# montyhall/bot7

Hardware: NVIDIA B200
Metric: EI candidates scored/s at N=4096, S=32 hypers (higher is better)
Workload: dtype f64

## Files before the change

bot7_b200/csrc/posterior_i8.cu:

```cuda
#include <math.h>
#include <stdlib.h>

#include "b7_internal.h"
#include "exp_neg.cuh"
#include "gemm_tile.cuh"
#include "i8_common.cuh"

using b7g::mbar_init; using b7g::mbar_wait; using b7g::mbar_arrive; using b7g::mbar_arrive_expect_tx; using b7g::bulk_g2s;
using b7g::mbar_fence_init; using b7g::smem_u32;
using namespace b7i8;

namespace {

constexpr int TM = 128, TN = 64, KB = 64;
constexpr int KC = KB / 16;
constexpr int A_STAGE = NS * TM * KB;
constexpr int B_STAGE = NS * TN * KB;
constexpr int STAGE = A_STAGE + B_STAGE;
constexpr int NSTAGE = 2;
static_assert(STAGE % 1024 == 0 && KB % 32 == 0 && 64 % KB == 0, "stage geometry");
static_assert(KB == b7i8::gemm::KB && TM == b7i8::gemm::TM && TN == b7i8::gemm::TN && NSTAGE == b7i8::gemm::NSTAGE,
              "posterior_i8_kernel issues its MMAs through the shared stage of i8_common.cuh");
constexpr int I8_THREADS = 192;
constexpr int RED_BYTES = 2 * 4 * TN * 8;
constexpr int I8_SMEM = NSTAGE * STAGE + RED_BYTES + 1024;
constexpr int TNH = TN / 2;
constexpr int B_HALF = NS * TNH * KB;
constexpr int P_STAGE = A_STAGE + B_HALF;
constexpr int P_NSTAGE = 3;
constexpr int P_SMEM = P_NSTAGE * P_STAGE + RED_BYTES + 1024;
constexpr int P_THREADS = 320;
static_assert(P_STAGE % 1024 == 0 && P_SMEM <= 227 * 1024, "pair stage geometry");


__host__ __device__ __forceinline__ long long pk_off(int rb) {
  const long long j = rb >> 1;
  return 4 * j * (j + 1) + (rb & 1) * 4 * (j + 1);
}

__global__ void __launch_bounds__(SLICE_THREADS)
slice_factor_kernel(const double* __restrict__ fac, long long fac_stride, int Np, int8_t* __restrict__ facS,
                    long long facS_stride, double* __restrict__ sigma, int s0) {
  __shared__ double s_red[SLICE_THREADS];
  const int rb = blockIdx.x, s = s0 + blockIdx.y, row = threadIdx.x & 127, q = threadIdx.x >> 7;
  const int KTA = Np / 16, NB = Np / TM;
  const int n_kc = rb < NB ? (rb + 1) * (TM / 16) : 0, all_kc = ((rb >> 1) + 1) * 4 * KC;
  int8_t* dst = facS + (long long)s * facS_stride + pk_off(rb) * A_STAGE;
  double inv = 0.0;
  const double* src = fac + (long long)s * fac_stride + b7g::tile_off(KTA, rb < NB ? rb : 0, 0);
  if (rb < NB) {
    double mx = 0.0;
    bool bad = false;
    for (int kc = q; kc < n_kc; kc += 4) chunk_max(src + b7g::elem_off(row, kc * 16), mx, bad);
    const double sg = row_scale(mx, bad, s_red, row, q);
    inv = sg != sg ? 0.0 : 1.0 / sg;
    if (q == 0) sigma[(long long)s * Np + rb * TM + row] = sg;
  }
  for (int kc = q; kc < all_kc; kc += 4) {
    uint32_t pk[4][NS];
    if (kc < n_kc) {
      chunk_digits(src + b7g::elem_off(row, kc * 16), inv, pk);
    } else {
#pragma unroll
      for (int g = 0; g < 4; ++g)
#pragma unroll
        for (int p = 0; p < NS; ++p) pk[g][p] = 0u;
    }
    const int ks = kc / KC, kcc = kc % KC;
#pragma unroll
    for (int p = 0; p < NS; ++p)
      *reinterpret_cast<uint4*>(dst + (long long)ks * A_STAGE + p * (KC * TM * 16) + kcc * (TM * 16) + row * 16) =
          make_uint4(pk[0][p], pk[1][p], pk[2][p], pk[3][p]);
  }
}

template <int DT, int KERNEL, bool PAIR>
__global__ void __launch_bounds__(128)
cov_slices_kernel(const double* __restrict__ A, long long rows, int d, const double* __restrict__ Xt, int N, int Np,
                  const double* __restrict__ par, double inv_tau, const double* __restrict__ alpha, int8_t* __restrict__ ksS,
                  double* __restrict__ meanP) {
  __shared__ __align__(16) double s_x[DT][64];
  __shared__ double s_w[DT];
  __shared__ double s_tab[64];
  __shared__ __align__(16) double s_al[64];
  __shared__ double s_dot[64];
  if (threadIdx.x < 64) s_tab[threadIdx.x] = c_exp_tab[threadIdx.x];
  const int ct = blockIdx.x, kb64 = blockIdx.y, KS_ALL = Np / KB;
  const int c = threadIdx.x & 63;
  for (int e = threadIdx.x; e < DT * 64; e += 128) {
    const int i = e / 64, k = kb64 * 64 + e % 64;
    s_x[i][e % 64] = (i < d && k < N) ? Xt[(long long)i * Np + k] : 0.0;
  }
  if (threadIdx.x >= 64) s_al[c] = alpha[kb64 * 64 + c];
  if (threadIdx.x < DT) s_w[threadIdx.x] = threadIdx.x < d ? par[threadIdx.x] : 0.0;
  __syncthreads();
  const long long row = (long long)ct * TN + c;
  double a[DT];
#pragma unroll
  for (int i = 0; i < DT; ++i) a[i] = (row < rows && i < d) ? A[row * d + i] : 0.0;
  const double sf2s = par[B7_MAX_DIMS] * inv_tau * 18014398509481984.0;
  double dot = 0.0;
  double w[DT];
#pragma unroll
  for (int j = 0; j < DT; ++j) w[j] = s_w[j];
  ExpNegK K;
  K.init();
  const bool live = row < rows;
#pragma unroll 1
  for (int half = 0; half < 2; ++half) {
  const int kc = (threadIdx.x >> 6) + 2 * half;
  uint32_t pk[4][NS];
  unsigned long long z[4];
#pragma unroll
  for (int i = 0; i < 16; i += 2) {
    const int kk = kc * 16 + i, k = kb64 * 64 + kk;
    double r2a = 0.0, r2b = 0.0;
#pragma unroll
    for (int j = 0; j < DT; ++j) {
      const double2 x2 = *reinterpret_cast<const double2*>(&s_x[j][kk]);
      const double ta = (a[j] - x2.x) * w[j], tb = (a[j] - x2.y) * w[j];
      r2a = fma(ta, ta, r2a);
      r2b = fma(tb, tb, r2b);
    }
    double va, vb;
    if (KERNEL == B7_KERNEL_ARDSE) {
      va = sf2s * exp_neg_k(-0.5 * r2a, s_tab, K);
      vb = sf2s * exp_neg_k(-0.5 * r2b, s_tab, K);
    } else {
      const double ra = sqrt(r2a), s5a = 2.23606797749978969641 * ra, rb = sqrt(r2b), s5b = 2.23606797749978969641 * rb;
      va = sf2s * ((1.0 + s5a + (5.0 / 3.0) * r2a) * exp_neg_k(-s5a, s_tab, K));
      vb = sf2s * ((1.0 + s5b + (5.0 / 3.0) * r2b) * exp_neg_k(-s5b, s_tab, K));
    }
    va = (live && k < N) ? va : 0.0;
    vb = (live && k + 1 < N) ? vb : 0.0;
    const double2 al = *reinterpret_cast<const double2*>(&s_al[kk]);
    dot = fma(va, al.x, dot);
    dot = fma(vb, al.y, dot);
    z[i & 3] = digit_bytes_scaled(va);
    z[(i & 3) + 1] = digit_bytes_scaled(vb);
    if ((i & 3) == 2) pack4(z, pk[i >> 2]);
  }
  const int gkc = kb64 * 4 + kc, ks = gkc / KC, kcc = gkc % KC;
  int8_t* dst = PAIR ? ksS + (((long long)ct * KS_ALL + ks) * 2 + (c >> 5)) * B_HALF + kcc * (TNH * 16) + (c & 31) * 16
                     : ksS + ((long long)ct * KS_ALL + ks) * B_STAGE + kcc * (TN * 16) + c * 16;
  constexpr int P_STRIDE = PAIR ? KC * TNH * 16 : KC * TN * 16;
#pragma unroll
  for (int p = 0; p < NS; ++p) *reinterpret_cast<uint4*>(dst + p * P_STRIDE) = make_uint4(pk[0][p], pk[1][p], pk[2][p], pk[3][p]);
  }
  if (threadIdx.x >= 64) s_dot[c] = dot;
  __syncthreads();
  if (threadIdx.x < 64) meanP[((long long)ct * (Np / 64) + kb64) * 64 + c] = dot + s_dot[c];
}

__device__ __forceinline__ double lane_transpose_sum(double (&x)[32], int lane) {
#pragma unroll
  for (int s = 16; s >= 1; s >>= 1) {
    const bool up = (lane & s) != 0;
#pragma unroll
    for (int j = 0; j < s; ++j) {
      const double send = up ? x[j] : x[j + s];
      const double keep = up ? x[j + s] : x[j];
      x[j] = keep + __shfl_xor_sync(0xffffffffu, send, s);
    }
  }
  return x[0];
}

struct Walk {
  int NB, chunk, group, n_tiles;
  __device__ __forceinline__ int cpt() const { return (NB + chunk - 1) / chunk; }
  __device__ __forceinline__ int npl() const { return (cpt() + 1) / 2; }
  __device__ __forceinline__ int n_items() const { return n_tiles * npl(); }
  __device__ __forceinline__ int grp(int item) const {
    const int g = item / (group * npl()), last = (n_tiles - 1) / group;
    return g < last ? g : last;
  }
  __device__ __forceinline__ int g_tiles(int g) const { return n_tiles - g * group < group ? n_tiles - g * group : group; }
  __device__ __forceinline__ int tile(int item) const {
    const int g = grp(item);
    return g * group + (item - g * group * npl()) % g_tiles(g);
  }
  __device__ __forceinline__ int level(int item) const {
    const int g = grp(item);
    return (item - g * group * npl()) / g_tiles(g);
  }
  __device__ __forceinline__ int parts(int item) const { return 2 * level(item) == cpt() - 1 ? 1 : 2; }
  __device__ __forceinline__ int rb_begin(int item, int part) const { return (part == 0 ? level(item) : cpt() - 1 - level(item)) * chunk; }
  __device__ __forceinline__ int rb_end(int item, int part) const {
    const int e = rb_begin(item, part) + chunk;
    return e < NB ? e : NB;
  }
};


template <typename F>
__device__ __forceinline__ void epilogue_row_block(uint32_t tmem, int tid, int warp, int lane, double sc, double* rr, double* out,
                                                   F arrive_drained) {
  double v[TN];
  b7i8::gemm::drain_classes(tmem, warp, v);
  tc_fence_before();
  __syncwarp();
  if (lane == 0) arrive_drained();
#pragma unroll
  for (int h = 0; h < 2; ++h) {
    double x[32];
#pragma unroll
    for (int c = 0; c < 32; ++c) { const double vv = v[h * 32 + c] * sc; x[c] = vv * vv; }
    rr[warp * TN + h * 32 + lane] = lane_transpose_sum(x, lane);
  }
  asm volatile("bar.sync 1, 128;\n" ::: "memory");
  if (tid < TN && out) out[tid] = ((rr[0 * TN + tid] + rr[1 * TN + tid]) + rr[2 * TN + tid]) + rr[3 * TN + tid];
}

template <typename F>
__device__ __forceinline__ void epilogue_row_block8(uint32_t tmem, int tid, int warp, int lane, double sc, double* rr, double* out,
                                                    F arrive_drained) {
  const int q = warp & 3, hc = warp >> 2;
  const uint32_t base = tmem + ((uint32_t)(q * 32) << 16) + (uint32_t)(hc * 32);
  double v[32];
  uint32_t a[4][32];
#pragma unroll
  for (int i = 0; i < 3; ++i) tmem_ld32_async(base + (uint32_t)(i * TN), a[i]);
  tmem_ld_wait();
#pragma unroll
  for (int c = 0; c < 32; ++c) v[c] = 0.0;
#pragma unroll
  for (int i = 0; i < 3; ++i) {
    tmem_pin(a[i]);
    const double wt = ldexp(1.0, 4 - 8 * (i + 2));
#pragma unroll
    for (int c = 0; c < 32; ++c) v[c] = fma((double)(int)a[i][c], wt, v[c]);
  }
#pragma unroll
  for (int i = 0; i < 4; ++i) tmem_ld32_async(base + (uint32_t)((3 + i) * TN), a[i]);
  tmem_ld_wait();
#pragma unroll
  for (int i = 0; i < 4; ++i) tmem_pin(a[i]);
  tc_fence_before();
  __syncwarp();
  if (lane == 0) arrive_drained();
#pragma unroll
  for (int i = 0; i < 4; ++i) {
    const double wt = ldexp(1.0, 4 - 8 * (i + 5));
#pragma unroll
    for (int c = 0; c < 32; ++c) v[c] = fma((double)(int)a[i][c], wt, v[c]);
  }
#pragma unroll
  for (int c = 0; c < 32; ++c) { const double vv = v[c] * sc; v[c] = vv * vv; }
  rr[q * TN + hc * 32 + lane] = lane_transpose_sum(v, lane);
  asm volatile("bar.sync 1, 256;\n" ::: "memory");
  if (tid < TN && out) out[tid] = ((rr[0 * TN + tid] + rr[1 * TN + tid]) + rr[2 * TN + tid]) + rr[3 * TN + tid];
}

__global__ void __launch_bounds__(I8_THREADS, 1)
posterior_i8_kernel(const int8_t* __restrict__ facS, const double* __restrict__ sigma, int Np, int NB,
                    const int8_t* __restrict__ ksS, double tau, int chunk, int group, int n_tiles, double* __restrict__ partial) {
  extern __shared__ __align__(1024) uint8_t smem[];
  double* red = reinterpret_cast<double*>(smem + NSTAGE * STAGE);
  uint64_t* bars = reinterpret_cast<uint64_t*>(smem + NSTAGE * STAGE + RED_BYTES);
  uint64_t *full = bars, *empty = bars + NSTAGE, *acc_full = bars + 2 * NSTAGE, *acc_empty = bars + 2 * NSTAGE + 1;
  uint32_t* tmem_slot = reinterpret_cast<uint32_t*>(bars + 2 * NSTAGE + 2);
  const int tid = threadIdx.x, warp = tid >> 5, lane = tid & 31;
  const int KS_ALL = Np / KB;
  const Walk wk{NB, chunk, group, n_tiles};
  if (tid == 0) {
    for (int s = 0; s < NSTAGE; ++s) { mbar_init(full + s, 1); mbar_init(empty + s, 1); }
    mbar_init(acc_full, 1);
    mbar_init(acc_empty, 4);
    mbar_fence_init();
  }
  if (warp == 4) {
    asm volatile("tcgen05.alloc.cta_group::1.sync.aligned.shared::cta.b32 [%0], %1;\n" ::"r"(smem_u32(tmem_slot)), "n"(512) : "memory");
    asm volatile("tcgen05.relinquish_alloc_permit.cta_group::1.sync.aligned;\n" ::: "memory");
  }
  tc_fence_before();
  __syncthreads();
  tc_fence_after();
  const uint32_t tmem = *tmem_slot;

  if (warp == 4) {
    int slot = 0;
    unsigned phase = 1;
    bool wrapped = false;
    for (int item = blockIdx.x; item < wk.n_items(); item += gridDim.x) {
      const int tile = wk.tile(item);
      const int8_t* gB = ksS + (long long)tile * KS_ALL * B_STAGE;
      for (int part = 0; part < wk.parts(item); ++part)
        for (int rb = wk.rb_begin(item, part); rb < wk.rb_end(item, part); ++rb) {
          const int8_t* gA = facS + pk_off(rb) * A_STAGE;
          for (int ks = 0; ks < (TM / KB) * (rb + 1); ++ks) {
            if (wrapped) mbar_wait(empty + slot, phase);
            if (elect_one()) {
              uint8_t* st = smem + slot * STAGE;
              mbar_arrive_expect_tx(full + slot, STAGE);
              bulk_g2s(st, gA + (long long)ks * A_STAGE, A_STAGE, full + slot);
              bulk_g2s(st + A_STAGE, gB + (long long)ks * B_STAGE, B_STAGE, full + slot);
            }
            __syncwarp();
            if (++slot == NSTAGE) { slot = 0; phase ^= 1u; wrapped = true; }
          }
        }
    }
  } else if (warp == 5) {
    const uint32_t idesc = (2u << 4) | (1u << 7) | (1u << 10) | ((uint32_t)(TN >> 3) << 17) | ((uint32_t)(TM >> 4) << 24);
    int slot = 0, done = 0;
    unsigned phase = 0;
    for (int item = blockIdx.x; item < wk.n_items(); item += gridDim.x)
      for (int part = 0; part < wk.parts(item); ++part)
        for (int rb = wk.rb_begin(item, part); rb < wk.rb_end(item, part); ++rb, ++done) {
          if (done > 0) { mbar_wait(acc_empty, (unsigned)((done - 1) & 1)); tc_fence_after(); }
          const int n_ks = (TM / KB) * (rb + 1);
          for (int ks = 0; ks < n_ks; ++ks) {
            mbar_wait(full + slot, phase);
            tc_fence_after();
            if (elect_one()) {
              b7i8::gemm::mma_stage(smem + slot * STAGE, tmem, idesc, ks == 0);
              umma_commit(empty + slot);
              if (ks == n_ks - 1) umma_commit(acc_full);
            }
            __syncwarp();
            if (++slot == NSTAGE) { slot = 0; phase ^= 1u; }
          }
        }
  } else {
    int done = 0;
    for (int item = blockIdx.x; item < wk.n_items(); item += gridDim.x) {
      const int tile = wk.tile(item);
      for (int part = 0; part < wk.parts(item); ++part)
        for (int rb = wk.rb_begin(item, part); rb < wk.rb_end(item, part); ++rb, ++done) {
          mbar_wait(acc_full, (unsigned)(done & 1));
          tc_fence_after();
          epilogue_row_block(tmem, tid, warp, lane, sigma[rb * TM + tid] * tau, red + (done & 1) * (4 * TN),
                             partial + ((long long)tile * NB + rb) * TN, [&] { mbar_arrive(acc_empty); });
        }
    }
  }
  tc_fence_before();
  __syncthreads();
  if (warp == 4) asm volatile("tcgen05.dealloc.cta_group::1.sync.aligned.b32 %0, %1;\n" ::"r"(tmem), "n"(512) : "memory");
}

__global__ void __cluster_dims__(2, 1, 1) __launch_bounds__(P_THREADS, 1)
posterior_i8_pair_kernel(const int8_t* __restrict__ facS, const double* __restrict__ sigma, int Np, int NB,
                         const int8_t* __restrict__ ksS, double tau, int group, int n_tiles, double* __restrict__ partial, int dbg) {
  extern __shared__ __align__(1024) uint8_t smem[];
  double* red = reinterpret_cast<double*>(smem + P_NSTAGE * P_STAGE);
  uint64_t* bars = reinterpret_cast<uint64_t*>(smem + P_NSTAGE * P_STAGE + RED_BYTES);
  uint64_t *full = bars, *empty = bars + P_NSTAGE, *peer_full = bars + 2 * P_NSTAGE, *acc_full = bars + 3 * P_NSTAGE,
           *acc_empty = bars + 3 * P_NSTAGE + 1;
  uint32_t* tmem_slot = reinterpret_cast<uint32_t*>(bars + 3 * P_NSTAGE + 2);
  const int tid = threadIdx.x, warp = tid >> 5, lane = tid & 31;
  const int KS_ALL = Np / KB;
  const uint32_t rank = cluster_ctarank();
  const int pair_id = blockIdx.x >> 1, n_pairs = gridDim.x >> 1;
  const Walk wk{(NB + 1) / 2, 1, group, n_tiles};
  if (tid == 0) {
    for (int s = 0; s < P_NSTAGE; ++s) { mbar_init(full + s, 1); mbar_init(empty + s, 1); mbar_init(peer_full + s, 1); }
    mbar_init(acc_full, 1);
    mbar_init(acc_empty, 16);
    mbar_fence_init();
  }
  if (warp == 8) {
    asm volatile("tcgen05.alloc.cta_group::2.sync.aligned.shared::cta.b32 [%0], %1;\n" ::"r"(smem_u32(tmem_slot)), "n"(512) : "memory");
    asm volatile("tcgen05.relinquish_alloc_permit.cta_group::2.sync.aligned;\n" ::: "memory");
  }
  tc_fence_before();
  __syncthreads();
  cluster_sync_all();
  tc_fence_after();
  const uint32_t tmem = *tmem_slot;

  if (warp == 8) {
    const uint64_t pol_last = l2_policy_evict_last(), pol_first = l2_policy_evict_first();
    int slot = 0;
    unsigned phase = 1;
    bool wrapped = false;
    for (int item = pair_id; item < wk.n_items(); item += n_pairs) {
      const int tile = wk.tile(item);
      const int8_t* gB = ksS + ((long long)tile * KS_ALL * 2 + rank) * B_HALF;
      for (int part = 0; part < wk.parts(item); ++part)
        for (int j = wk.rb_begin(item, part); j < wk.rb_end(item, part); ++j) {
          const int8_t* gA = facS + pk_off(2 * j + (int)rank) * A_STAGE;
          for (int ks = 0; ks < 4 * (j + 1); ++ks) {
            if (wrapped) mbar_wait_cluster(empty + slot, phase);
            if (elect_one()) {
              uint8_t* st = smem + slot * P_STAGE;
              if (dbg & 4) {
                mbar_arrive_expect_tx(full + slot, 2048);
                bulk_g2s(st, facS, 1024, full + slot);
                bulk_g2s(st + A_STAGE, ksS, 1024, full + slot);
                __syncwarp();
                if (++slot == P_NSTAGE) { slot = 0; phase ^= 1u; wrapped = true; }
                continue;
              }
              mbar_arrive_expect_tx(full + slot, P_STAGE);
              if (dbg & 2) {
                bulk_g2s(st, facS, A_STAGE, full + slot);
                bulk_g2s(st + A_STAGE, ksS, B_HALF, full + slot);
              } else {
                const int hint = dbg >> 4;
                if (hint == 1 || hint == 2) bulk_g2s_hint(st, gA + (long long)ks * A_STAGE, A_STAGE, full + slot, pol_last);
                else if (hint == 4 || hint == 5) bulk_g2s_hint(st, gA + (long long)ks * A_STAGE, A_STAGE, full + slot, pol_first);
                else bulk_g2s(st, gA + (long long)ks * A_STAGE, A_STAGE, full + slot);
                if (hint == 2 || hint == 3) bulk_g2s_hint(st + A_STAGE, gB + (long long)ks * (2 * B_HALF), B_HALF, full + slot, pol_first);
                else if (hint == 4 || hint == 6) bulk_g2s_hint(st + A_STAGE, gB + (long long)ks * (2 * B_HALF), B_HALF, full + slot, pol_last);
                else bulk_g2s(st + A_STAGE, gB + (long long)ks * (2 * B_HALF), B_HALF, full + slot);
              }
            }
            __syncwarp();
            if (++slot == P_NSTAGE) { slot = 0; phase ^= 1u; wrapped = true; }
          }
        }
    }
  } else if (warp == 9) {
    int slot = 0, done = 0;
    unsigned phase = 0;
    if (rank == 0) {
      const uint32_t idesc = (2u << 4) | (1u << 7) | (1u << 10) | ((uint32_t)(TN >> 3) << 17) | ((uint32_t)(256 >> 4) << 24);
      for (int item = pair_id; item < wk.n_items(); item += n_pairs)
        for (int part = 0; part < wk.parts(item); ++part)
          for (int j = wk.rb_begin(item, part); j < wk.rb_end(item, part); ++j, ++done) {
            if (done > 0) { mbar_wait_cluster(acc_empty, (unsigned)((done - 1) & 1)); tc_fence_after(); }
            const int n_ks = 4 * (j + 1);
            for (int ks = 0; ks < n_ks; ++ks) {
              mbar_wait_cluster(full + slot, phase);
              mbar_wait_cluster(peer_full + slot, phase);
              tc_fence_after();
              if (elect_one()) {
                const uint8_t* st = smem + slot * P_STAGE;
                const uint64_t da0 = umma_desc(st, TM * 16, 128), db0 = umma_desc(st + A_STAGE, TNH * 16, 128);
#pragma unroll
                for (int k2 = 0; k2 < KB / 32; ++k2) {
#pragma unroll
                  for (int p = 1; p <= NS; ++p) {
                    const uint64_t da = da0 + (uint64_t)(((p - 1) * (KC * TM * 16) + k2 * (2 * TM * 16)) >> 4);
                    const uint32_t acc = (ks == 0 && k2 == 0 && p == 1) ? 0u : 1u;
                    const int nq = NS + 1 - p;
#pragma unroll
                    for (int q = 1; q <= nq; ++q) {
                      const uint64_t db = db0 + (uint64_t)(((q - 1) * (KC * TNH * 16) + k2 * (2 * TNH * 16)) >> 4);
                      const uint32_t dcol = tmem + (uint32_t)((p + q - 2) * TN);
                      if (nq == 1) umma_i8_pair<0>(dcol, da, db, idesc, acc);
                      else if (q == 1) umma_i8_pair<1>(dcol, da, db, idesc, acc);
                      else if (q == nq) umma_i8_pair<3>(dcol, da, db, idesc, acc);
                      else umma_i8_pair<2>(dcol, da, db, idesc, acc);
                    }
                  }
                }
                umma_commit_pair(empty + slot);
                if (ks == n_ks - 1) umma_commit_pair(acc_full);
              }
              __syncwarp();
              if (++slot == P_NSTAGE) { slot = 0; phase ^= 1u; }
            }
          }
    } else {
      for (int item = pair_id; item < wk.n_items(); item += n_pairs)
        for (int part = 0; part < wk.parts(item); ++part)
          for (int j = wk.rb_begin(item, part); j < wk.rb_end(item, part); ++j)
            for (int ks = 0; ks < 4 * (j + 1); ++ks) {
              mbar_wait_cluster(full + slot, phase);
              if (elect_one()) mbar_arrive_cluster(peer_full + slot, 0);
              __syncwarp();
              if (++slot == P_NSTAGE) { slot = 0; phase ^= 1u; }
            }
    }
  } else {
    int done = 0;
    for (int item = pair_id; item < wk.n_items(); item += n_pairs) {
      const int tile = wk.tile(item);
      for (int part = 0; part < wk.parts(item); ++part)
        for (int j = wk.rb_begin(item, part); j < wk.rb_end(item, part); ++j, ++done) {
          const int rb = 2 * j + (int)rank;
          mbar_wait_cluster(acc_full, (unsigned)(done & 1));
          tc_fence_after();
          if (dbg & 1) {
            tc_fence_before();
            __syncwarp();
            if (lane == 0) mbar_arrive_cluster(acc_empty, 0);
            continue;
          }
          const double sc = rb < NB ? sigma[rb * TM + (tid & 127)] * tau : 0.0;
          epilogue_row_block8(tmem, tid, warp, lane, sc, red + (done & 1) * (4 * TN),
                             rb < NB ? partial + ((long long)tile * NB + rb) * TN : nullptr, [&] { mbar_arrive_cluster(acc_empty, 0); });
        }
    }
  }
  tc_fence_before();
  __syncthreads();
  cluster_sync_all();
  if (warp == 8) asm volatile("tcgen05.dealloc.cta_group::2.sync.aligned.b32 %0, %1;\n" ::"r"(tmem), "n"(512) : "memory");
}

__global__ void __launch_bounds__(128)
posterior_i8_finish_kernel(const double* __restrict__ partial, const double* __restrict__ meanP, int NB, int Np,
                           const double* __restrict__ cand, long long rows, int d, const double* __restrict__ Xt,
                           const double* __restrict__ par, int kernel, double sf2, double mconst, double mean_scale,
                           long long cols_pad, double* __restrict__ mean, double* __restrict__ var) {
  const long long c = (long long)blockIdx.x * blockDim.x + threadIdx.x;
  if (c >= cols_pad) return;
  const double* p = partial + (c / TN) * NB * TN + c % TN;
  double run2 = 0.0, run1 = 0.0;
  for (int rb = 0; rb < NB; ++rb) run2 += p[(long long)rb * TN];
  const double* q = meanP + (c / TN) * (Np / 64) * 64 + c % TN;
  for (int kb = 0; kb < Np / 64; ++kb) run1 += q[(long long)kb * 64];
  double r2 = 0.0;
  if (c < rows)
    for (int j = 0; j < d; ++j) {
      const double t = (cand[c * d + j] - Xt[(long long)j * Np]) * par[j];
      r2 = fma(t, t, r2);
    }
  const bool nan_row = (r2 != r2) || (kernel == B7_KERNEL_MATERN52 && isinf(r2));
  const double poison = nan_row ? __longlong_as_double(0x7ff8000000000000LL) : 0.0;
  const double vv = sf2 - run2;
  var[c] = (vv > 0.0 ? vv : (vv != vv ? vv : 0.0)) + poison;
  mean[c] = (nan_row ? 0.0 : fma(run1, mean_scale, mconst)) + poison;
}

bool g_attr_i8[16] = {false};

}

size_t b7_i8_facs_stride(int Np) {
  const long long P = (Np / TM + 1) / 2;
  return (size_t)(4 * P * (P + 1)) * A_STAGE;
}

int b7_i8_slice_factor(b7_ctx* ctx, const double* fac, int Np, int8_t* facS, double* sigma, int s0, int count) {
  const int NBp = (Np / TM + 1) / 2 * 2;
  slice_factor_kernel<<<dim3(NBp, count), SLICE_THREADS, 0, ctx->stream>>>(fac, (long long)Np * Np, Np, facS, (long long)b7_i8_facs_stride(Np), sigma, s0);
  b7_count(ctx);
  B7_CUDA(cudaGetLastError());
  return 0;
}

template <int DT>
static int launch_cov_slices(b7_ctx* ctx, cudaStream_t st, int kernel, const double* A, int64_t rows, int64_t rows_pad, int d,
                             const double* Xt, int N, int Np, const double* par, double inv_tau, const double* alpha, int8_t* ksS,
                             double* meanP) {
  dim3 grid((unsigned)(rows_pad / TN), Np / 64);
  const bool se = kernel == B7_KERNEL_ARDSE;
  if (ctx->post_pair) {
    if (se) cov_slices_kernel<DT, B7_KERNEL_ARDSE, true><<<grid, 128, 0, st>>>(A, rows, d, Xt, N, Np, par, inv_tau, alpha, ksS, meanP);
    else cov_slices_kernel<DT, B7_KERNEL_MATERN52, true><<<grid, 128, 0, st>>>(A, rows, d, Xt, N, Np, par, inv_tau, alpha, ksS, meanP);
  } else {
    if (se) cov_slices_kernel<DT, B7_KERNEL_ARDSE, false><<<grid, 128, 0, st>>>(A, rows, d, Xt, N, Np, par, inv_tau, alpha, ksS, meanP);
    else cov_slices_kernel<DT, B7_KERNEL_MATERN52, false><<<grid, 128, 0, st>>>(A, rows, d, Xt, N, Np, par, inv_tau, alpha, ksS, meanP);
  }
  b7_count(ctx);
  B7_CUDA(cudaGetLastError());
  return 0;
}

int b7_i8_cov_slices(b7_ctx* ctx, cudaStream_t st, int kernel, const double* A, int64_t rows, int64_t rows_pad, int d, const double* Xt,
                     int N, int Np, const double* par, double tau, const double* alpha, int8_t* ksS, double* meanP) {
  if (rows_pad <= 0) return 0;
  const double inv_tau = 1.0 / tau;
#define B7_COV_SLICES(DT) return launch_cov_slices<DT>(ctx, st, kernel, A, rows, rows_pad, d, Xt, N, Np, par, inv_tau, alpha, ksS, meanP)
  if (d <= 2) B7_COV_SLICES(2);
  if (d <= 4) B7_COV_SLICES(4);
  if (d <= 6) B7_COV_SLICES(6);
  if (d <= 8) B7_COV_SLICES(8);
  if (d <= 12) B7_COV_SLICES(12);
  if (d <= 16) B7_COV_SLICES(16);
  if (d <= 20) B7_COV_SLICES(20);
  if (d <= 24) B7_COV_SLICES(24);
  if (d <= 32) B7_COV_SLICES(32);
  B7_COV_SLICES(40);
#undef B7_COV_SLICES
}

size_t b7_i8_partial_bytes(int Np, int64_t cols_pad) {
  return (size_t)(cols_pad / TN) * ((size_t)(Np / TM) * TN + (size_t)(Np / 64) * 64) * sizeof(double);
}
double* b7_i8_mean_partials(double* partial, int Np, int64_t cols_pad) { return partial + (size_t)(cols_pad / TN) * (Np / TM) * TN; }

int b7_launch_posterior_i8(b7_ctx* ctx, const int8_t* facS, const double* sigma, int Np, const int8_t* ksS, const double* cand,
                           int64_t rows, int d, const double* Xt, const double* par, int kernel, int64_t cols_pad, double tau,
                           double sf2, double mconst, double* partial, double* mean, double* var) {
  if (!g_attr_i8[ctx->device & 15]) {
    B7_CUDA(cudaFuncSetAttribute(posterior_i8_kernel, cudaFuncAttributeMaxDynamicSharedMemorySize, I8_SMEM));
    B7_CUDA(cudaFuncSetAttribute(posterior_i8_pair_kernel, cudaFuncAttributeMaxDynamicSharedMemorySize, P_SMEM));
    g_attr_i8[ctx->device & 15] = true;
  }
  if (cols_pad <= 0) return 0;
  const int NB = Np / TM;
  static const int group_env = getenv("B7_POST_GROUP") ? atoi(getenv("B7_POST_GROUP")) : 0;
  const int n_tiles = (int)(cols_pad / TN), group = group_env > 0 ? group_env : 16;
  if (ctx->post_pair) {
    const int P = (NB + 1) / 2, n_items = n_tiles * ((P + 1) / 2), n_pairs = ctx->sm_count / 2;
    static const int dbg_env = getenv("B7_POST_DBG") ? atoi(getenv("B7_POST_DBG")) : 0;
    posterior_i8_pair_kernel<<<2 * (n_items < n_pairs ? n_items : n_pairs), P_THREADS, P_SMEM, ctx->stream>>>(facS, sigma, Np, NB, ksS, tau, group,
                                                                                                              n_tiles, partial, dbg_env);
  } else {
    static const int chunk_env = getenv("B7_POST_CHUNK") ? atoi(getenv("B7_POST_CHUNK")) : 0;
    const int chunk = chunk_env > 0 ? (chunk_env < NB ? chunk_env : NB) : (NB < 2 ? NB : 2);
    const int cpt = (NB + chunk - 1) / chunk;
    const int n_items = n_tiles * ((cpt + 1) / 2);
    posterior_i8_kernel<<<n_items < ctx->sm_count ? n_items : ctx->sm_count, I8_THREADS, I8_SMEM, ctx->stream>>>(facS, sigma, Np, NB, ksS, tau, chunk,
                                                                                                                group, n_tiles, partial);
  }
  posterior_i8_finish_kernel<<<(unsigned)((cols_pad + 127) / 128), 128, 0, ctx->stream>>>(partial, b7_i8_mean_partials(partial, Np, cols_pad), NB, Np,
                                                                                         cand, rows, d, Xt, par, kernel, sf2, mconst,
                                                                                         tau * 5.5511151231257827e-17, cols_pad, mean, var);
  b7_count(ctx, 2);
  B7_CUDA(cudaGetLastError());
  return 0;
}
```

Measured before the change: 181,500.

## Pipeline TMEM accumulator per class slot to overlap epilogue with next MMA block

Replaces the single acc_full/acc_empty handshake in the cluster-pair posterior kernel with per-class ready barriers and per-slot empty barriers. The TMEM column slots are remapped across alternating row blocks, so the next block's MMAs can start writing a class slot as soon as the epilogue has drained it. The aim is to remove the stall where the MMA warp waited for the whole accumulator to be drained before starting the next row block. This adds more mbarrier traffic and more complex phase tracking, and it relies on the slot-aliasing logic being correct.

```diff
diff --git a/bot7_b200/csrc/posterior_i8.cu b/bot7_b200/csrc/posterior_i8.cu
--- a/bot7_b200/csrc/posterior_i8.cu
+++ b/bot7_b200/csrc/posterior_i8.cu
@@ -212,38 +212,30 @@
   if (tid < TN && out) out[tid] = ((rr[0 * TN + tid] + rr[1 * TN + tid]) + rr[2 * TN + tid]) + rr[3 * TN + tid];
 }
 
-template <typename F>
-__device__ __forceinline__ void epilogue_row_block8(uint32_t tmem, int tid, int warp, int lane, double sc, double* rr, double* out,
-                                                    F arrive_drained) {
+__device__ __forceinline__ int class_slot(int w, bool odd) { return !odd ? w - 2 : (w == NS + 1 ? NS : NS - w); }
+
+__device__ __forceinline__ void epilogue_row_block8(uint32_t tmem, int tid, int warp, int lane, bool odd, unsigned par, uint64_t* ready,
+                                                    uint64_t* slot_empty, double sc, double* rr, double* out) {
   const int q = warp & 3, hc = warp >> 2;
   const uint32_t base = tmem + ((uint32_t)(q * 32) << 16) + (uint32_t)(hc * 32);
   double v[32];
-  uint32_t a[4][32];
-#pragma unroll
-  for (int i = 0; i < 3; ++i) tmem_ld32_async(base + (uint32_t)(i * TN), a[i]);
-  tmem_ld_wait();
 #pragma unroll
   for (int c = 0; c < 32; ++c) v[c] = 0.0;
 #pragma unroll
-  for (int i = 0; i < 3; ++i) {
-    tmem_pin(a[i]);
-    const double wt = ldexp(1.0, 4 - 8 * (i + 2));
-#pragma unroll
-    for (int c = 0; c < 32; ++c) v[c] = fma((double)(int)a[i][c], wt, v[c]);
-  }
-#pragma unroll
-  for (int i = 0; i < 4; ++i) tmem_ld32_async(base + (uint32_t)((3 + i) * TN), a[i]);
-  tmem_ld_wait();
-#pragma unroll
-  for (int i = 0; i < 4; ++i) tmem_pin(a[i]);
-  tc_fence_before();
-  __syncwarp();
-  if (lane == 0) arrive_drained();
-#pragma unroll
-  for (int i = 0; i < 4; ++i) {
-    const double wt = ldexp(1.0, 4 - 8 * (i + 5));
-#pragma unroll
-    for (int c = 0; c < 32; ++c) v[c] = fma((double)(int)a[i][c], wt, v[c]);
+  for (int w = 2; w <= NS + 1; ++w) {
+    const int s = class_slot(w, odd);
+    uint32_t a[32];
+    mbar_wait_cluster(ready + (w - 2), par);
+    tc_fence_after();
+    tmem_ld32_async(base + (uint32_t)(s * TN), a);
+    tmem_ld_wait();
+    tmem_pin(a);
+    tc_fence_before();
+    __syncwarp();
+    if (lane == 0) mbar_arrive_cluster(slot_empty + s, 0);
+    const double wt = ldexp(1.0, 4 - 8 * w);
+#pragma unroll
+    for (int c = 0; c < 32; ++c) v[c] = fma((double)(int)a[c], wt, v[c]);
   }
 #pragma unroll
   for (int c = 0; c < 32; ++c) { const double vv = v[c] * sc; v[c] = vv * vv; }
@@ -340,15 +332,31 @@
   if (warp == 4) asm volatile("tcgen05.dealloc.cta_group::1.sync.aligned.b32 %0, %1;\n" ::"r"(tmem), "n"(512) : "memory");
 }
 
+__device__ __forceinline__ void pair_group(const uint8_t* st, int p, int k2, const uint32_t (&col)[NS], uint32_t idesc, uint32_t acc1) {
+  const uint64_t da = umma_desc(st, TM * 16, 128) + (uint64_t)(((p - 1) * (KC * TM * 16) + k2 * (2 * TM * 16)) >> 4);
+  const uint64_t db0 = umma_desc(st + A_STAGE, TNH * 16, 128);
+  const int nq = NS + 1 - p;
+#pragma unroll
+  for (int q = 1; q <= nq; ++q) {
+    const uint64_t db = db0 + (uint64_t)(((q - 1) * (KC * TNH * 16) + k2 * (2 * TNH * 16)) >> 4);
+    const uint32_t dcol = col[p + q - 2];
+    const uint32_t acc = q == 1 ? acc1 : 1u;
+    if (nq == 1) umma_i8_pair<0>(dcol, da, db, idesc, acc);
+    else if (q == 1) umma_i8_pair<1>(dcol, da, db, idesc, acc);
+    else if (q == nq) umma_i8_pair<3>(dcol, da, db, idesc, acc);
+    else umma_i8_pair<2>(dcol, da, db, idesc, acc);
+  }
+}
+
 __global__ void __cluster_dims__(2, 1, 1) __launch_bounds__(P_THREADS, 1)
 posterior_i8_pair_kernel(const int8_t* __restrict__ facS, const double* __restrict__ sigma, int Np, int NB,
                          const int8_t* __restrict__ ksS, double tau, int group, int n_tiles, double* __restrict__ partial, int dbg) {
   extern __shared__ __align__(1024) uint8_t smem[];
   double* red = reinterpret_cast<double*>(smem + P_NSTAGE * P_STAGE);
   uint64_t* bars = reinterpret_cast<uint64_t*>(smem + P_NSTAGE * P_STAGE + RED_BYTES);
-  uint64_t *full = bars, *empty = bars + P_NSTAGE, *peer_full = bars + 2 * P_NSTAGE, *acc_full = bars + 3 * P_NSTAGE,
-           *acc_empty = bars + 3 * P_NSTAGE + 1;
-  uint32_t* tmem_slot = reinterpret_cast<uint32_t*>(bars + 3 * P_NSTAGE + 2);
+  uint64_t *full = bars, *empty = bars + P_NSTAGE, *peer_full = bars + 2 * P_NSTAGE, *ready = bars + 3 * P_NSTAGE,
+           *slot_empty = ready + NS;
+  uint32_t* tmem_slot = reinterpret_cast<uint32_t*>(slot_empty + NS + 1);
   const int tid = threadIdx.x, warp = tid >> 5, lane = tid & 31;
   const int KS_ALL = Np / KB;
   const uint32_t rank = cluster_ctarank();
@@ -356,8 +364,8 @@
   const Walk wk{(NB + 1) / 2, 1, group, n_tiles};
   if (tid == 0) {
     for (int s = 0; s < P_NSTAGE; ++s) { mbar_init(full + s, 1); mbar_init(empty + s, 1); mbar_init(peer_full + s, 1); }
-    mbar_init(acc_full, 1);
-    mbar_init(acc_empty, 16);
+    for (int w = 0; w < NS; ++w) mbar_init(ready + w, 1);
+    for (int s = 0; s <= NS; ++s) mbar_init(slot_empty + s, 16);
     mbar_fence_init();
   }
   if (warp == 8) {
@@ -414,41 +422,51 @@
     }
   } else if (warp == 9) {
     int slot = 0, done = 0;
-    unsigned phase = 0;
+    unsigned phase = 0, slot_wait = 0, slot_par = 0;
     if (rank == 0) {
       const uint32_t idesc = (2u << 4) | (1u << 7) | (1u << 10) | ((uint32_t)(TN >> 3) << 17) | ((uint32_t)(256 >> 4) << 24);
       for (int item = pair_id; item < wk.n_items(); item += n_pairs)
         for (int part = 0; part < wk.parts(item); ++part)
           for (int j = wk.rb_begin(item, part); j < wk.rb_end(item, part); ++j, ++done) {
-            if (done > 0) { mbar_wait_cluster(acc_empty, (unsigned)((done - 1) & 1)); tc_fence_after(); }
             const int n_ks = 4 * (j + 1);
+            const bool odd = done & 1;
+            uint32_t col[NS];
+#pragma unroll
+            for (int w = 2; w <= NS + 1; ++w) col[w - 2] = tmem + (uint32_t)(class_slot(w, odd) * TN);
             for (int ks = 0; ks < n_ks; ++ks) {
               mbar_wait_cluster(full + slot, phase);
               mbar_wait_cluster(peer_full + slot, phase);
               tc_fence_after();
+              const uint8_t* st = smem + slot * P_STAGE;
+              if (ks == 0) {
+#pragma unroll
+                for (int k2 = 0; k2 < KB / 32; ++k2)
+#pragma unroll
+                  for (int p = NS; p >= 1; --p) {
+                    if (k2 == 0) {
+                      const int s = class_slot(p + 1, odd);
+                      if ((slot_wait >> s) & 1u) {
+                        mbar_wait_cluster(slot_empty + s, (slot_par >> s) & 1u);
+                        slot_par ^= 1u << s;
+                        tc_fence_after();
+                      }
+                      slot_wait |= 1u << s;
+                    }
+                    if (elect_one()) pair_group(st, p, k2, col, idesc, k2 == 0 ? 0u : 1u);
+                    __syncwarp();
+                  }
+              }
               if (elect_one()) {
-                const uint8_t* st = smem + slot * P_STAGE;
-                const uint64_t da0 = umma_desc(st, TM * 16, 128), db0 = umma_desc(st + A_STAGE, TNH * 16, 128);
-#pragma unroll
-                for (int k2 = 0; k2 < KB / 32; ++k2) {
-#pragma unroll
-                  for (int p = 1; p <= NS; ++p) {
-                    const uint64_t da = da0 + (uint64_t)(((p - 1) * (KC * TM * 16) + k2 * (2 * TM * 16)) >> 4);
-                    const uint32_t acc = (ks == 0 && k2 == 0 && p == 1) ? 0u : 1u;
-                    const int nq = NS + 1 - p;
-#pragma unroll
-                    for (int q = 1; q <= nq; ++q) {
-                      const uint64_t db = db0 + (uint64_t)(((q - 1) * (KC * TNH * 16) + k2 * (2 * TNH * 16)) >> 4);
-                      const uint32_t dcol = tmem + (uint32_t)((p + q - 2) * TN);
-                      if (nq == 1) umma_i8_pair<0>(dcol, da, db, idesc, acc);
-                      else if (q == 1) umma_i8_pair<1>(dcol, da, db, idesc, acc);
-                      else if (q == nq) umma_i8_pair<3>(dcol, da, db, idesc, acc);
-                      else umma_i8_pair<2>(dcol, da, db, idesc, acc);
+                if (ks > 0) {
+#pragma unroll
+                  for (int k2 = 0; k2 < KB / 32; ++k2)
+#pragma unroll
+                    for (int p = 1; p <= NS; ++p) {
+                      pair_group(st, p, k2, col, idesc, 1u);
+                      if (ks == n_ks - 1 && k2 == KB / 32 - 1) umma_commit_pair(ready + (p - 1));
                     }
-                  }
                 }
                 umma_commit_pair(empty + slot);
-                if (ks == n_ks - 1) umma_commit_pair(acc_full);
               }
               __syncwarp();
               if (++slot == P_NSTAGE) { slot = 0; phase ^= 1u; }
@@ -472,17 +490,20 @@
       for (int part = 0; part < wk.parts(item); ++part)
         for (int j = wk.rb_begin(item, part); j < wk.rb_end(item, part); ++j, ++done) {
           const int rb = 2 * j + (int)rank;
-          mbar_wait_cluster(acc_full, (unsigned)(done & 1));
-          tc_fence_after();
+          const bool odd = done & 1;
           if (dbg & 1) {
-            tc_fence_before();
-            __syncwarp();
-            if (lane == 0) mbar_arrive_cluster(acc_empty, 0);
+            for (int w = 2; w <= NS + 1; ++w) {
+              mbar_wait_cluster(ready + (w - 2), (unsigned)(done & 1));
+              tc_fence_after();
+              tc_fence_before();
+              __syncwarp();
+              if (lane == 0) mbar_arrive_cluster(slot_empty + class_slot(w, odd), 0);
+            }
             continue;
           }
           const double sc = rb < NB ? sigma[rb * TM + (tid & 127)] * tau : 0.0;
-          epilogue_row_block8(tmem, tid, warp, lane, sc, red + (done & 1) * (4 * TN),
-                             rb < NB ? partial + ((long long)tile * NB + rb) * TN : nullptr, [&] { mbar_arrive_cluster(acc_empty, 0); });
+          epilogue_row_block8(tmem, tid, warp, lane, odd, (unsigned)(done & 1), ready, slot_empty, sc, red + (done & 1) * (4 * TN),
+                             rb < NB ? partial + ((long long)tile * NB + rb) * TN : nullptr);
         }
     }
   }
```

New measurement: 174,600 (median of 6 runs). -3.8%, worse.
